# sea-sky-web/Vision-based-Spatio-Temporal-Analysis

Hardware: AMD Instinct MI355X
Metric: multi-cam frames/sec (7-cam→480×1440 BEV) (higher is better)
Workload: dtype f32; 1 GPU; 7-cam 1080x1920 -> resnet50(stride-8 features)+proj C=64 -> IPM warp -> mean -> 480x1440 BEV (BASELINE configs[1]); cameras=7, cameras_per_gpu=7, channels=64, bev_memory_format=NCHW, parallelism=frame-sharded x1 (no collective)

## Files before the change

include/bev_mi355x.h:

```cpp
#ifndef BEV_MI355X_H
#define BEV_MI355X_H

#include <stdint.h>

#ifdef __cplusplus
extern "C" {
#endif

#define BEV_ERR_ARGS (-1)

#define BEV_FUSE_SUM 0
#define BEV_FUSE_MEAN 1
#define BEV_FUSE_MAX 2

int bev_abi_version(void);

const char *bev_build_source_hash(void);

#define BEV_TUNE_CONV_TILE 1
#define BEV_TUNE_WARP_POOL_KB 2
#define BEV_TUNE_WARP_KERNEL 3
#define BEV_TUNE_WARP_BWD_POOL 5
#define BEV_TUNE_CONV_XCD 6
#define BEV_TUNE_CONV_NBUF 7
#define BEV_TUNE_WGRAD_MFMA 8
#define BEV_TUNE_CONV_DMA 9
#define BEV_TUNE_CONV_X6_TILE 10
#define BEV_TUNE_CONV_X6_KERNEL 11
#define BEV_TUNE_CONV_H16_KERNEL 12
#define BEV_TUNE_CONV_PW_SMALL 13
#define BEV_TUNE_DW_RUN 14
#define BEV_TUNE_CONV_X6_NT 16
#define BEV_TUNE_STEM3_STAGE 17
#define BEV_TUNE_WARP_SPAN 19
#define BEV_TUNE_WARP_TILE_BAND 20
#define BEV_TUNE_CONV_H16_BUF 21
int bev_tune(int knob, int value);


int bev_linspace_f32(double lo, double hi, int n, float *out_host);

int bev_homography_f32(const float *K, const float *G, int n, float *H, void *stream);


int bev_ipm_warp_f32(const float *feats, int64_t sN, int64_t sC, int64_t sH, int64_t sW, const float *Hmat,
                     const float *xs, const float *ys, int N, int C, int Hf, int Wf, float sx, float sy, int Hb,
                     int Wb, float *out, void *stream);

int bev_ipm_warp_fuse_f32(const float *feats, int64_t sN, int64_t sC, int64_t sH, int64_t sW, const float *Hmat,
                          const float *xs, const float *ys, int B, int V, int C, int Hf, int Wf, float sx, float sy,
                          int Hb, int Wb, int mode, float *out, void *stream);

int64_t bev_ipm_warp_fuse_workspace_bytes(int B, int V, int Hb, int Wb);
int bev_ipm_warp_fuse_ws_f32(const float *feats, int64_t sN, int64_t sC, int64_t sH, int64_t sW, const float *Hmat,
                             const float *xs, const float *ys, int B, int V, int C, int Hf, int Wf, float sx, float sy,
                             int Hb, int Wb, int mode, float *out, void *workspace, int64_t workspace_bytes,
                             void *stream);
int bev_ipm_warp_fuse_boxes_f32(const float *Hmat, const float *xs, const float *ys, int B, int V, int Hf, int Wf,
                                float sx, float sy, int Hb, int Wb, int mode, void *workspace, int64_t workspace_bytes,
                                void *stream);
int bev_ipm_warp_fuse_pre_f32(const float *feats, int64_t sN, int64_t sC, int64_t sH, int64_t sW, const float *Hmat,
                              const float *xs, const float *ys, int B, int V, int C, int Hf, int Wf, float sx, float sy,
                              int Hb, int Wb, int mode, float *out, void *workspace, int64_t workspace_bytes,
                              void *stream);
int bev_ipm_warp_fuse_nhwc_f32(const float *feats, int64_t sN, int64_t sC, int64_t sH, int64_t sW, const float *Hmat,
                               const float *xs, const float *ys, int B, int V, int C, int Hf, int Wf, float sx,
                               float sy, int Hb, int Wb, int mode, float *out, void *workspace,
                               int64_t workspace_bytes, int boxes_ready, void *stream);
int bev_ipm_warp_fuse_chunked_f32(const float *feats, int64_t sN, int64_t sC, int64_t sH, int64_t sW,
                                  const float *Hmat, const float *xs, const float *ys, int B, int V, int C, int Hf,
                                  int Wf, float sx, float sy, int Hb, int Wb, int mode, int rows_per_chunk, float *out,
                                  void *workspace, int64_t workspace_bytes, int boxes_ready, void *stream);

int bev_ipm_taps_f32(const float *Hmat, const float *xs, const float *ys, int N, int Hf, int Wf, float sx, float sy,
                     int Hb, int Wb, int32_t *x0y0, float *wts, uint8_t *valid, void *stream);

int bev_ipm_warp_bwd_f32(const float *gout, const float *Hmat, const float *xs, const float *ys, int N, int C, int Hf,
                         int Wf, float sx, float sy, int Hb, int Wb, float *gfeats, void *stream);

int bev_ipm_warp_bwd_ex_f32(const float *gout, const float *Hmat, const float *xs, const float *ys, int N, int C,
                            int Hf, int Wf, float sx, float sy, int Hb, int Wb, float *gfeats, int64_t sN, int64_t sC,
                            int64_t sH, int64_t sW, void *stream);

int bev_ipm_warp_fuse_bwd_f32(const float *gout, const float *Hmat, const float *xs, const float *ys, int B, int V,
                              int C, int Hf, int Wf, float sx, float sy, int Hb, int Wb, int mode, float *gfeats,
                              void *stream);

int bev_ipm_warp_fuse_bwd_ex_f32(const float *gout, const float *Hmat, const float *xs, const float *ys, int B,
                                 int V, int C, int Hf, int Wf, float sx, float sy, int Hb, int Wb, int mode,
                                 float *gfeats, int64_t sN, int64_t sC, int64_t sH, int64_t sW, void *stream);

int bev_view_fuse_f32(const float *x, int B, int V, int64_t M, int mode, float *out, void *stream);

int bev_view_max_bwd_f32(const float *x, const float *gout, int B, int V, int64_t M, float *gx, void *stream);


int64_t bev_conv_packed_size(int Co, int Ci, int KH, int KW);

int bev_conv_pack_weights_f32(const float *w, int Co, int Ci, int KH, int KW, float *packed, void *stream);

int bev_conv2d_f32(const float *x, int in_nchw, int N, int H, int W, int Ci, const float *packed, const float *bias,
                   const float *residual, int Co, int KH, int KW, int stride, int pad, int relu, float *y, int Ho,
                   int Wo, void *stream);

int bev_conv2d_chscale_f32(const float *x, int N, int H, int W, int Ci, const float *gate, const float *packed,
                           const float *bias, const float *residual, int Co, int KH, int KW, int stride, int pad,
                           int relu, float *y, int Ho, int Wo, void *stream);

int bev_conv2d_dual_f32(const float *x, int N, int Ho, int Wo, int Ci, const float *x2, int H2, int W2, int Ci2,
                        int stride2, const float *packed, const float *bias, int Co, int relu, float *y,
                        void *stream);

int bev_conv2d_chain_f32(const float *x, int N, int H, int W, int Ci, const float *packed, const float *bias, int Co,
                         int KH, int KW, int stride, int pad, int relu, const float *packed2, const float *bias2,
                         int Co2, const float *residual, int relu2, float *y, int Ho, int Wo, void *stream);

int bev_conv2d_chain_dual_f32(const float *x, int N, int H, int W, int Ci, const float *packed, const float *bias,
                              int Co, int KH, int KW, int stride, int pad, int relu, const float *x2, int H2, int W2,
                              int Ci2, int stride2, const float *packed2, const float *bias2, int Co2, int relu2,
// ... 297 lines not shown
```

vision-based-spatio-temporal-analysis_amd/bev_native.py:

```python
from __future__ import annotations

import collections.abc
import contextlib
import ctypes
import functools
import os
import subprocess
import threading

import torch

HERE = os.path.dirname(os.path.abspath(__file__))
LIB_PATH = os.path.join(HERE, "libbev_mi355x.so")
ABI_VERSION = 18
BEV_ERR_ARGS = -1

FUSE_MODES = {"sum": 0, "mean": 1, "max": 2}

_lib = None

_vp = ctypes.c_void_p
_i = ctypes.c_int
_i64 = ctypes.c_int64
_f = ctypes.c_float
# ... 164 lines not shown
    global _SPANS
    spans, _SPANS = _SPANS or {}, None
    torch.cuda.synchronize()
    return {k: [a.elapsed_time(b) for a, b in v] for k, v in spans.items()}


@contextlib.contextmanager
def _span(name: str, t: torch.Tensor):
    if _SPANS is None:
        yield
        return
    st = torch.cuda.current_stream(t.device)
    e0, e1 = torch.cuda.Event(enable_timing=True), torch.cuda.Event(enable_timing=True)
    e0.record(st)
    yield
    e1.record(st)
    _SPANS.setdefault(name, []).append((e0, e1))


def build(force: bool = False) -> str:
    cmd = ["make", "-s", "-C", HERE] + (["-B"] if force else [])
    subprocess.check_call(cmd)
    return LIB_PATH


def lib():
    global _lib
    if _lib is None:
        if not os.path.exists(LIB_PATH):
            raise ImportError(f"libbev_mi355x.so not built ({LIB_PATH}); run __graft_entry__.build()")
        L = ctypes.CDLL(LIB_PATH)
        for name, (res, args) in SIGNATURES.items():
            fn = getattr(L, name)
            fn.restype = res
            fn.argtypes = args
        v = L.bev_abi_version()
        if v != ABI_VERSION:
            raise ImportError(f"libbev_mi355x.so ABI {v} != expected {ABI_VERSION}; rebuild")
        _lib = L
    return _lib


def source_hash() -> str:
    import hashlib
    mk = open(os.path.join(HERE, "Makefile")).read()
    files = []
    for var in ("SRCS", "HDRS"):
        line = next(l for l in mk.splitlines() if l.startswith(var + " ="))
        files += line.split("=", 1)[1].split()
    h = hashlib.sha256()
    for f in files:
        with open(os.path.join(HERE, f), "rb") as fh:
            h.update(fh.read())
    return h.hexdigest()[:16]


def provenance() -> dict:
    built = lib().bev_build_source_hash().decode()
    try:
        tree = source_hash()
    except OSError:
        tree = None
    return {"lib": LIB_PATH, "lib_source_hash": built, "tree_source_hash": tree, "matches_tree": built == tree}


TUNE_CONV_TILE = 1
TUNE_WARP_POOL_KB = 2
TUNE_WARP_KERNEL = 3
TUNE_WARP_BWD_POOL = 5
TUNE_CONV_XCD = 6
TUNE_CONV_NBUF = 7
TUNE_WGRAD_MFMA = 8
TUNE_CONV_DMA = 9
TUNE_CONV_X6_TILE = 10
TUNE_CONV_X6_KERNEL = 11
TUNE_CONV_H16_KERNEL = 12
TUNE_CONV_PW_SMALL = 13
TUNE_DW_RUN = 14
TUNE_CONV_X6_NT = 16
TUNE_STEM3_STAGE = 17
TUNE_WARP_SPAN = 19
TUNE_WARP_TILE_BAND = 20
TUNE_CONV_H16_BUF = 21
WARP_KERNEL_DMA, WARP_KERNEL_REGISTER = 0, 1


def tune(knob: int, value: int) -> int:
    rc = lib().bev_tune(knob, value)
    if rc < 0:
        raise ValueError(f"bad tuning knob/value {knob}/{value}")
    return rc


@contextlib.contextmanager
def tuned(**knobs):
    old = []
    try:
        for name, value in knobs.items():
            k = globals()["TUNE_" + name]
            old.append((k, tune(k, value)))
        yield
    finally:
        for k, v in reversed(old):
            tune(k, v)


class HipError(RuntimeError):
    pass


AMP_HALF_CONVS = True
_AMP_LOCAL = threading.local()


CONV_ARITHS = ("f32", "bf16x6", "f16")
_ARITH = {"mode": "bf16x6"}


def conv_arith() -> str:
    return _ARITH["mode"]


def set_conv_arith(mode: str) -> str:
    if mode not in CONV_ARITHS:
        raise ValueError(f"conv arithmetic {mode!r} not in {CONV_ARITHS}")
    prev, _ARITH["mode"] = _ARITH["mode"], mode
    return prev


@contextlib.contextmanager
def conv_arith_mode(mode: str):
    prev = set_conv_arith(mode)
    try:
        yield
    finally:
        set_conv_arith(prev)


HEAD_ARITHS = ("f32", "f16")
_HEAD_ARITH = {"mode": "f32"}


def head_arith() -> str:
    return _HEAD_ARITH["mode"]


def set_head_arith(mode: str) -> str:
    if mode not in HEAD_ARITHS:
        raise ValueError(f"head arithmetic {mode!r} not in {HEAD_ARITHS}")
    prev, _HEAD_ARITH["mode"] = _HEAD_ARITH["mode"], mode
    return prev


@contextlib.contextmanager
def head_arith_mode(mode: str):
    prev = set_head_arith(mode)
    try:
        yield
    finally:
        set_head_arith(prev)


def half_convs() -> bool:
    return getattr(_AMP_LOCAL, "half", False)


# ... 1842 lines not shown
```

vision-based-spatio-temporal-analysis_amd/csrc/bev_conv.hip:

```cpp
#include <hip/hip_runtime.h>
#include <stdint.h>
#include <stdlib.h>

#include <type_traits>

#include "../../include/bev_mi355x.h"
#include "bev_act.h"
#include "bev_mfma.h"
#include "bev_tune.h"

namespace {

constexpr int BK = 32;
constexpr int LROW = BK + 4;

typedef float f32x16 __attribute__((ext_vector_type(16)));
typedef float f32x2 __attribute__((ext_vector_type(2)));
typedef float f32x4 __attribute__((ext_vector_type(4)));

__device__ __attribute__((aligned(16))) float g_zero4[4] = {0.f, 0.f, 0.f, 0.f};

__host__ __device__ inline int64_t kpad(int K) { return (K + BK - 1) / BK * BK; }
__host__ __device__ inline int64_t copad(int Co) { return (Co + 127) / 128 * 128; }

// ... 1189 lines not shown
        default: return false;
    }
    rc = last();
    return true;
}

int g_conv_tile = 0;

int g_conv_xcd = 1;
int g_conv_nbuf = 0;
inline int conv_xcd() { return g_conv_xcd; }

int launch_tiled(const ConvArgs &a, int loader, hipStream_t st) {
    int rc_pw = 0;
    if (g_conv_tile == 0 && try_pw_small(a, loader, st, rc_pw)) return rc_pw;
    if (g_conv_tile == 0 && try_pw_mfma(a, loader, st, rc_pw)) return rc_pw;
    const int64_t M = a.M;
    const int Co = a.Co;
    const int nbuf_env = g_conv_nbuf;
    auto nbuf1_for = [&](int tile) {
        if (nbuf_env == 1 || nbuf_env == 2) return nbuf_env == 1;
        return tile == 3 || M >= 400000;
    };
    int tile = g_conv_tile;
    if (tile == 0) {
        auto cost = [&](int bm, int bn, int resident) {
            const int64_t blocks = ((M + bm - 1) / bm) * ((Co + bn - 1) / bn);
            return (double)((blocks + resident - 1) / resident) * bm * bn;
        };
        const double c1 = cost(128, 128, 512), c3 = cost(64, 128, nbuf1_for(3) ? 768 : 512),
                     c2 = cost(128, 64, nbuf1_for(2) ? 768 : 512);
        tile = 1;
        double best = c1;
        if (c3 < 0.95 * best) { tile = 3; best = c3; }
        if (c2 < 0.95 * best) { tile = 2; best = c2; }
        if (a.KH == 1 && a.KW == 1 && (loader == 1 || loader == 6) && M >= 200000) tile = 4;
        if (a.KH == 1 && a.KW == 1 && loader == 4 && M >= 200000 && (Co <= 64 || a.Ci >= 48)) tile = 4;
    }
    if (tile == 2)
        return nbuf1_for(2) ? launch_conv<4, 1, 1, 2, 1>(a, loader, st) : launch_conv<4, 1, 1, 2>(a, loader, st);
    if (tile == 3)
        return nbuf1_for(3) ? launch_conv<2, 2, 1, 2, 1>(a, loader, st) : launch_conv<2, 2, 1, 2>(a, loader, st);
    if (tile == 4) return launch_conv<2, 2, 1, 1, 1>(a, loader, st);
    return launch_conv<2, 2, 2, 2>(a, loader, st);
}

int launch_chain(const ConvArgs &a, hipStream_t st) {
    const int bm = a.Co == 64 ? 128 : 64;
    const int64_t blocks = (a.M + bm - 1) / bm;
    if (blocks > 0x7fffffff) return BEV_ERR_ARGS;
    const dim3 g((unsigned)blocks), b(256);
    if (use_dma(a.Co)) {
        if (a.Co == 64) hipLaunchKernelGGL((k_conv_dma<4, 1, 1, 2, 1>), g, b, 0, st, a);
        else hipLaunchKernelGGL((k_conv_dma<2, 2, 1, 2, 1>), g, b, 0, st, a);
    } else if (a.Co == 64) hipLaunchKernelGGL((k_conv<4, 1, 1, 2, 1, 1, 1>), g, b, 0, st, a);
    else hipLaunchKernelGGL((k_conv<2, 2, 1, 2, 1, 1, 1>), g, b, 0, st, a);
    return last();
}

ConvArgs conv_args(const float *x, const float *packed, const float *bias, const float *res, float *y, int N, int H,
                   int W, int Ci, int Co, int KH, int KW, int stride, int pad, int dil, int Ho, int Wo, int relu,
                   int ldy) {
    ConvArgs a;
    a.x = x, a.wp = packed, a.bias = bias, a.res = res, a.y = y;
    a.N = N, a.H = H, a.W = W, a.Ci = Ci, a.Co = Co, a.KH = KH, a.KW = KW, a.stride = stride, a.pad = pad;
    a.dil = dil, a.Ho = Ho, a.Wo = Wo, a.relu = relu, a.ldy = ldy;
    a.M = (int64_t)N * Ho * Wo;
    a.K = Ci * KH * KW;
    a.Kp = (int)kpad(a.K);
    a.xcd = conv_xcd();
    return a;
}

}

extern "C" {

int bev_tune(int knob, int value) {
    if (knob == BEV_TUNE_CONV_TILE) return bev::swap_knob(g_conv_tile, value, 4);
    if (knob == BEV_TUNE_CONV_DMA) return bev::swap_knob(g_conv_dma, value, 2);
    if (knob == BEV_TUNE_CONV_XCD) return bev::swap_knob(g_conv_xcd, value, 1);
    if (knob == BEV_TUNE_CONV_NBUF) return bev::swap_knob(g_conv_nbuf, value, 2);
    if (knob == BEV_TUNE_WGRAD_MFMA) return bev::train_tune(knob, value);
    if (knob == BEV_TUNE_CONV_X6_TILE || knob == BEV_TUNE_CONV_X6_KERNEL || knob == BEV_TUNE_CONV_X6_NT)
        return bev::conv_x6_tune(knob, value);
    if (knob == BEV_TUNE_CONV_H16_KERNEL) return bev::conv_h16_tune(value);
    if (knob == BEV_TUNE_CONV_H16_BUF) return bev::conv_h16_buf_tune(value);
    if (knob == BEV_TUNE_DW_RUN) return bev::dw_tune(value);
    if (knob == BEV_TUNE_STEM3_STAGE) return bev::stem3_tune(value);
    if (knob == BEV_TUNE_CONV_PW_SMALL) return bev::swap_knob(g_conv_pw_small, value, 4);
    return bev::warp_tune(knob, value);
}

int64_t bev_conv_packed_size(int Co, int Ci, int KH, int KW) {
    if (Co <= 0 || Ci <= 0 || KH <= 0 || KW <= 0) return 0;
    return copad(Co) * kpad(Ci * KH * KW);
}

int bev_conv_pack_weights_f32(const float *w, int Co, int Ci, int KH, int KW, float *packed, void *stream) {
    if (!w || !packed || Co <= 0 || Ci <= 0 || KH <= 0 || KW <= 0) return BEV_ERR_ARGS;
    const int64_t Kp = kpad(Ci * KH * KW), Cop = copad(Co);
    const int64_t total = Kp * Cop;
    hipLaunchKernelGGL(k_pack, dim3((unsigned)((total + 255) / 256)), dim3(256), 0, (hipStream_t)stream, w, Co, Ci,
                       KH, KW, Kp, Cop, packed);
    return last();
}

static int conv2d_impl(const float *x, int in_nchw, int N, int H, int W, int Ci, const float *packed,
                       const float *bias, const float *residual, int Co, int KH, int KW, int stride, int pad, int relu,
                       float *y, int Ho, int Wo, const float *ascale, void *stream, int dil, int ldy,
                       const float *ashift, int arelu);

int bev_conv2d_f32(const float *x, int in_nchw, int N, int H, int W, int Ci, const float *packed, const float *bias,
                   const float *residual, int Co, int KH, int KW, int stride, int pad, int relu, float *y, int Ho,
                   int Wo, void *stream) {
    return conv2d_impl(x, in_nchw, N, H, W, Ci, packed, bias, residual, Co, KH, KW, stride, pad, relu, y, Ho, Wo,
                       nullptr, stream, 1, Co, nullptr, 0);
}

int bev_conv2d_nhwc_ex_f32(const float *x, int N, int H, int W, int Ci, const float *in_scale, const float *in_shift,
                           int in_relu, const float *packed, const float *bias, int Co, int KH, int KW, int stride,
                           int pad, int dilation, int relu, float *y, int ldy, int Ho, int Wo, void *stream) {
    if ((in_shift || in_relu) && !in_scale) return BEV_ERR_ARGS;
    if (in_scale && (Ci % BK != 0 || ((((uintptr_t)in_scale) | ((uintptr_t)in_shift) | ((uintptr_t)x)) & 15) != 0))
        return BEV_ERR_ARGS;
    return conv2d_impl(x, 0, N, H, W, Ci, packed, bias, nullptr, Co, KH, KW, stride, pad, relu, y, Ho, Wo, in_scale,
                       stream, dilation, ldy, in_shift, in_relu != 0);
}

int bev_conv2d_chscale_f32(const float *x, int N, int H, int W, int Ci, const float *gate, const float *packed,
                           const float *bias, const float *residual, int Co, int KH, int KW, int stride, int pad,
                           int relu, float *y, int Ho, int Wo, void *stream) {
    if (!gate || ((((uintptr_t)gate) | ((uintptr_t)x)) & 15) != 0 || Ci % 4 != 0) return BEV_ERR_ARGS;
    const bool fast = Ci % BK == 0;
    const bool contig = KH == 1 && KW == 1 && stride == 1 && pad == 0;
    if (!fast && !contig) return BEV_ERR_ARGS;
    return conv2d_impl(x, 0, N, H, W, Ci, packed, bias, residual, Co, KH, KW, stride, pad, relu, y, Ho, Wo, gate,
                       stream, 1, Co, nullptr, 0);
}

static int conv2d_impl(const float *x, int in_nchw, int N, int H, int W, int Ci, const float *packed,
                       const float *bias, const float *residual, int Co, int KH, int KW, int stride, int pad, int relu,
                       float *y, int Ho, int Wo, const float *ascale, void *stream, int dil, int ldy,
                       const float *ashift, int arelu) {
    if (!x || !packed || !y || N < 0 || H <= 0 || W <= 0 || Ci <= 0 || Co <= 0 || KH <= 0 || KW <= 0 ||
        stride <= 0 || pad < 0 || relu < 0 || relu > 2 || dil <= 0 || ldy < Co || (residual && ldy != Co))
        return BEV_ERR_ARGS;
    if (Ho != conv_out(H, pad, dil, KH, stride) || Wo != conv_out(W, pad, dil, KW, stride) ||
        Ho <= 0 || Wo <= 0)
        return BEV_ERR_ARGS;
    if (N == 0) return 0;
    ConvArgs a = conv_args(x, packed, bias, residual, y, N, H, W, Ci, Co, KH, KW, stride, pad, dil, Ho, Wo, relu, ldy);
    a.in_nchw = in_nchw;
    const bool pw = !in_nchw && KH == 1 && KW == 1 && stride == 1 && pad == 0 && Ci % 4 == 0 &&
                    ((uintptr_t)x & 15) == 0;
    int loader = (!in_nchw && Ci % BK == 0) ? 1 : (in_nchw && Ci == 3 && KH == 7 && KW == 7) ? 2 : pw ? 4 : 0;
    if (loader == 1 && (ashift || arelu || dil != 1)) loader = 5;
    else if (loader == 1 && ascale) loader = 6;
    if ((ashift || arelu) && loader != 5) return BEV_ERR_ARGS;
    a.ascale = ascale;
    a.ashift = ashift;
    a.arelu = arelu;
    if (in_nchw && Ci == 3 && KH == 7 && KW == 7 && stride == 2 && pad == 3 && Co <= 64 && !residual && bias &&
        g_conv_tile == 0 && relu <= 1 && !ascale && dil == 1 && ldy == Co)
        return launch_stem(x, N, H, W, packed, a.Kp, bias, Co, y, Ho, Wo, relu, (hipStream_t)stream);
    return launch_tiled(a, loader, (hipStream_t)stream);
}
// ... 169 lines not shown
```

vision-based-spatio-temporal-analysis_amd/csrc/bev_conv_x6.hip:

```cpp
#include <hip/hip_runtime.h>
#include <stdint.h>

#include <type_traits>

#include "../../include/bev_mi355x.h"
#include "bev_act.h"
#include "bev_mfma.h"
#include "bev_tune.h"

namespace {

typedef __bf16 bf16x8 __attribute__((ext_vector_type(8)));
typedef __bf16 bf16x4 __attribute__((ext_vector_type(4)));
typedef float f32x16 __attribute__((ext_vector_type(16)));
typedef float f32x4 __attribute__((ext_vector_type(4)));
typedef unsigned u32x4 __attribute__((ext_vector_type(4)));
typedef unsigned u32x2 __attribute__((ext_vector_type(2)));

constexpr int XBK = 16;
constexpr int XROW = 24;

__device__ __attribute__((aligned(16))) float g_xzero4[4] = {0.f, 0.f, 0.f, 0.f};

__host__ __device__ inline int64_t kpad_x(int K) { return (K + XBK - 1) / XBK * XBK; }
// ... 611 lines not shown
            *(bf16x4 *)(d + 2 * APL) = lv;                                                                 \
        }                                                                                                  \
    } while (0)
#define X6B_BLOAD(BS, G)                                                                                   \
    do {                                                                                                   \
        const int g_ = (G) < nslice ? (G) : nslice - 1;              \
        _Pragma("unroll") for (int j = 0; j < TN; ++j)                                                     \
            _Pragma("unroll") for (int p = 0; p < 3; ++p)                                                  \
                BS[j][p] = *(const bf16x8 *)(wb + ((int64_t)j * S + g_) * 1536 + p * 512);                \
    } while (0)
    const int r32 = lane & 31, h = lane >> 5;
#define X6B_SLICE(AS, KK, BC)                                                                              \
    do {                                                                                                   \
        bf16x8 fa[TM][3];                                                                                  \
        _Pragma("unroll") for (int i = 0; i < TM; ++i)                                                     \
            _Pragma("unroll") for (int p = 0; p < 3; ++p)                                                  \
                fa[i][p] = *(const bf16x8 *)(AS + p * APL + (wm * TM * 32 + i * 32 + r32) * YROW + 16 * (KK) + 8 * h); \
        _Pragma("unroll") for (int i = 0; i < TM; ++i)                                                     \
            _Pragma("unroll") for (int j = 0; j < TN; ++j)                                                 \
                x6_dot(acc[i][j], fa[i], BC[j]);                                                           \
    } while (0)
#define X6B_MFMA(BUF, KS)                                                                                  \
    do {                                                                                                   \
        const __bf16 *As = lds + (BUF) * STAGE;                                                            \
        X6B_SLICE(As, 0, bs0);                                                                             \
        X6B_BLOAD(bs0, 2 * (KS) + 2);                                                                      \
        X6B_SLICE(As, 1, bs1);                                                                             \
    } while (0)

    const int nk = a.Kp / YBK;
    X6B_BLOAD(bs0, 0);
    X6B_GLOAD(va0);
    if (nk > 1) X6B_GLOAD(va1);
    X6B_SWRITE(0, va0);
    __syncthreads();
    int ks = 0;
    for (; ks + 3 < nk; ks += 2) {
        X6B_BLOAD(bs1, 2 * ks + 1);
        X6B_GLOAD(va0);
        X6B_MFMA(0, ks);
        X6B_SWRITE(1, va1);
        __syncthreads();
        X6B_BLOAD(bs1, 2 * ks + 3);
        X6B_GLOAD(va1);
        X6B_MFMA(1, ks + 1);
        X6B_SWRITE(0, va0);
        __syncthreads();
    }
    if (ks + 2 < nk) {
        X6B_BLOAD(bs1, 2 * ks + 1);
        X6B_GLOAD(va0);
        X6B_MFMA(0, ks);
        X6B_SWRITE(1, va1);
        __syncthreads();
        X6B_BLOAD(bs1, 2 * ks + 3);
        X6B_MFMA(1, ks + 1);
        X6B_SWRITE(0, va0);
        __syncthreads();
        X6B_BLOAD(bs1, 2 * ks + 5);
        X6B_MFMA(0, ks + 2);
    } else if (ks + 1 < nk) {
        X6B_BLOAD(bs1, 2 * ks + 1);
        X6B_MFMA(0, ks);
        X6B_SWRITE(1, va1);
        __syncthreads();
        X6B_BLOAD(bs1, 2 * ks + 3);
        X6B_MFMA(1, ks + 1);
    } else {
        X6B_BLOAD(bs1, 2 * ks + 1);
        X6B_MFMA(0, ks);
    }
#undef X6B_MFMA
#undef X6B_SLICE
#undef X6B_BLOAD
#undef X6B_SWRITE
#undef X6B_GLOAD
    if constexpr (CHAIN > 0) {
        x6_chain_epilogue<WM, WN, TM, TN, CHAIN == 2 ? 4 : 0>(a, lds_raw, acc, wave, lane, wm, wn, m0);
        return;
    }
    x6_epilogue<TM, TN>(a, (float *)lds_raw, acc, wave, lane, wn, wm, m0, n0);
}

template <int WM, int WN, int TM, int TN, int CHAIN = 0>
__global__ __launch_bounds__(256, CHAIN ? 2 : 3) void k_conv_x6s(ConvX a) {
    constexpr bool BLDS = CHAIN > 0;
    constexpr int BM = WM * TM * 32, BN = WN * TN * 32;
    constexpr int APL = BM * 32;
    constexpr int BST = BLDS ? BN / 32 * 6 * 512 : 0;
    constexpr int STAGE = 3 * APL + BST;
    constexpr int RW = BM / 4;
    constexpr int RG = RW / 16;
    constexpr int BPW = BLDS ? BN / 32 * 6 / 4 : 0;
    constexpr int EPIB = CHAIN ? x6_chain_lds_bytes<BM, BN>() : x6_epi_bytes<TN>();
    constexpr int LDSB = (2 * STAGE * 2 > EPIB) ? 2 * STAGE * 2 : EPIB;
    static_assert(RW % 16 == 0, "whole DMA groups per wave");
    static_assert(!BLDS || (BN / 32 * 6) % 4 == 0, "whole B pieces per wave");
    __shared__ __attribute__((aligned(16))) unsigned char lds_raw[LDSB];
    const __bf16 *lds = (const __bf16 *)lds_raw;

    const int tid = threadIdx.x;
    const int lane = tid & 63, wave = __builtin_amdgcn_readfirstlane(tid >> 6);
    const int wm = wave / WN, wn = wave % WN;
    const int n_tiles = (a.Co + BN - 1) / BN;
    const unsigned bid = xcd_block(blockIdx.x, gridDim.x);
    const int64_t m0 = (int64_t)(bid / n_tiles) * BM;
    const int n0 = (bid % n_tiles) * BN;

    int64_t abase[RG];
    int aiy[RG], aix[RG];
    bool aok[RG];
#pragma unroll
    for (int g = 0; g < RG; ++g) {
        const int row = wave * RW + 16 * g + (lane >> 2);
        const int lc = (lane & 3) ^ ((row >> 2) & 3);
        const int64_t m = m0 + row;
        aok[g] = m < a.M;
        const int64_t mm = aok[g] ? m : 0;
        const int ox = (int)(mm % a.Wo);
        const int64_t t = mm / a.Wo;
        const int oy = (int)(t % a.Ho);
        const int64_t n = t / a.Ho;
        aiy[g] = oy * a.stride - a.pad;
        aix[g] = ox * a.stride - a.pad;
        abase[g] = ((n * a.H + aiy[g]) * a.W + aix[g]) * a.Ci + 8 * lc;
    }
    const unsigned lbase = (unsigned)__builtin_amdgcn_readfirstlane((int)lds_addr(lds_raw));
    const int S = a.Kp / XBK;
    int ky = 0, kx = 0, ci0 = 0, kstep = 0;
    const __bf16 *bsrc = a.wp + (int64_t)(n0 >> 5) * S * 1536 + lane * 8;
    auto issue = [&](int buf) {
        if constexpr (BLDS) {
            const unsigned db = lbase + (unsigned)(buf * STAGE * 2 + 3 * APL * 2);
#pragma unroll
            for (int i = 0; i < BPW; ++i) {
                const int q = wave + 4 * i, cbl = q / 6, r = q % 6;
                lds_dma16(bsrc + ((int64_t)cbl * S + 2 * kstep + r / 3) * 1536 + (r % 3) * 512,
                      db + (unsigned)(q * 1024));
            }
            ++kstep;
        }
        const int64_t toff = ((int64_t)ky * a.dil * a.W + kx * a.dil) * a.Ci + ci0;
        const unsigned d0 = lbase + (unsigned)(buf * STAGE * 2) + (unsigned)(wave * RW * 64);
#pragma unroll
        for (int g = 0; g < RG; ++g) {
            const int iy = aiy[g] + ky * a.dil, ix = aix[g] + kx * a.dil;
            const bool in = aok[g] && (unsigned)iy < (unsigned)a.H && (unsigned)ix < (unsigned)a.W;
            const __bf16 *src = a.xs + abase[g] + toff;
#pragma unroll
            for (int p = 0; p < 3; ++p)
                lds_dma16(in ? (const void *)(src + p * a.xps) : (const void *)g_xzero4,
                      d0 + (unsigned)(p * APL * 2 + g * 1024));
        }
        ci0 += YBK;
        if (ci0 == a.Ci) {
            ci0 = 0;
            if (++kx == a.KW) {
                kx = 0;
                ++ky;
            }
        }
    };

    const __amdgpu_buffer_rsrc_t rw = buffer_rsrc(a.wp, copad_x(a.Co) / 32 * (int64_t)S * 3072);
    const int cb0 = (n0 + wn * TN * 32) >> 5;
    const int vl = lane * 16;
    bf16x8 bs0[TN][3], bs1[TN][3];
#define X6S_BLOAD(BS, G)                                                                                   \
    do {                                                                                                   \
        const int g_ = (G) < S ? (G) : S - 1;                                                              \
        _Pragma("unroll") for (int j = 0; j < TN; ++j)                                                     \
            _Pragma("unroll") for (int p = 0; p < 3; ++p)                                                  \
                BS[j][p] = __builtin_bit_cast(                                                             \
                    bf16x8, __builtin_amdgcn_raw_buffer_load_b128(rw, vl, (((cb0 + j) * S + g_) * 3 + p) * 1024, 0)); \
    } while (0)
    const int r32 = lane & 31, h = lane >> 5;
#define X6S_SLICE(AS, KK, BC)                                                                              \
    do {                                                                                                   \
        bf16x8 fa[TM][3];                                                                                  \
        _Pragma("unroll") for (int i = 0; i < TM; ++i) {                                                   \
            const int R = wm * TM * 32 + i * 32 + r32;                                                     \
            const int ph = (2 * (KK) + h) ^ ((R >> 2) & 3);                                                \
            _Pragma("unroll") for (int p = 0; p < 3; ++p)                                                  \
                fa[i][p] = *(const bf16x8 *)(AS + p * APL + R * 32 + ph * 8);                              \
        }                                                                                                  \
        _Pragma("unroll") for (int i = 0; i < TM; ++i)                                                     \
            _Pragma("unroll") for (int j = 0; j < TN; ++j)                                                 \
                x6_dot(acc[i][j], fa[i], BC[j]);                                                           \
    } while (0)

    f32x16 acc[TM][TN];
#pragma unroll
    for (int i = 0; i < TM; ++i)
#pragma unroll
        for (int j = 0; j < TN; ++j) acc[i][j] = (f32x16){0};
    const int nk = a.Kp / YBK;
    if constexpr (BLDS) {
        issue(0);
        asm volatile("s_waitcnt vmcnt(0)" ::: "memory");
        __syncthreads();
        for (int ks = 0; ks < nk; ++ks) {
            const int cur = ks & 1;
            if (ks + 1 < nk) issue(cur ^ 1);
            const __bf16 *As = lds + cur * STAGE;
            const __bf16 *Bs = As + 3 * APL + lane * 8;
#pragma unroll
            for (int kk = 0; kk < 2; ++kk) {
                bf16x8 fb[TN][3];
#pragma unroll
                for (int j = 0; j < TN; ++j)
#pragma unroll
                    for (int p = 0; p < 3; ++p) fb[j][p] = *(const bf16x8 *)(Bs + (((wn * TN + j) * 2 + kk) * 3 + p) * 512);
                X6S_SLICE(As, kk, fb);
            }
            asm volatile("s_waitcnt vmcnt(0)" ::: "memory");
            __syncthreads();
        }
    } else {
        X6S_BLOAD(bs0, 0);
        issue(0);
        asm volatile("s_waitcnt vmcnt(0)" ::: "memory");
        __syncthreads();
        for (int ks = 0; ks < nk; ++ks) {
            const int cur = ks & 1;
            if (ks + 1 < nk) issue(cur ^ 1);
            const __bf16 *As = lds + cur * STAGE;
            X6S_BLOAD(bs1, 2 * ks + 1);
            X6S_SLICE(As, 0, bs0);
            X6S_BLOAD(bs0, 2 * ks + 2);
            X6S_SLICE(As, 1, bs1);
            asm volatile("s_waitcnt vmcnt(0)" ::: "memory");
            __syncthreads();
        }
    }
#undef X6S_SLICE
#undef X6S_BLOAD
    if constexpr (CHAIN > 0) {
        x6_chain_epilogue<WM, WN, TM, TN, CHAIN == 2 ? 4 : 0>(a, lds_raw, acc, wave, lane, wm, wn, m0);
        return;
    }
    x6_epilogue<TM, TN>(a, (float *)lds_raw, acc, wave, lane, wn, wm, m0, n0);
}

__global__ void k_split3(const float *__restrict__ x, int64_t n, __bf16 *__restrict__ out) {
    const int64_t t = (int64_t)blockIdx.x * blockDim.x + threadIdx.x;
    if (t >= n) return;
    __bf16 h, m, l;
    split3(x[t], h, m, l);
    out[t] = h;
    out[t + n] = m;
    out[t + 2 * n] = l;
}

int g_x6_tile = 0;
int g_x6_nt = 0;
int g_x6_kernel = 0;

int launch_x6(void (*kernel)(ConvX), int BM, int BN, const ConvX &a, hipStream_t st) {
    const int64_t blocks = ((a.M + BM - 1) / BM) * ((a.Co + BN - 1) / BN);
    if (blocks >= ((int64_t)1 << 31)) return BEV_ERR_ARGS;
    hipLaunchKernelGGL(kernel, dim3((unsigned)blocks), dim3(256), 0, st, a);
    return last();
}

enum X6Form { X6_PLAIN, X6_DUAL, X6_CHAIN, X6_CHAIN_DUAL };
struct X6Call {
    X6Form form;
    const float *x = nullptr;
    const uint16_t *xs = nullptr, *packed = nullptr;
    const float *bias = nullptr, *res = nullptr;
    float *y = nullptr;
    uint16_t *ys = nullptr;
    int N = 0, H = 0, W = 0, Ci = 0, Co = 0, KH = 1, KW = 1, stride = 1, pad = 0, dil = 1, act = 0, ldy = 0, Ho = 0,
        Wo = 0;
    const float *x2 = nullptr;
    int H2 = 0, W2 = 0, Ci2 = 0, stride2 = 0;
    const uint16_t *packed2 = nullptr;
    const float *bias2 = nullptr;
    int Co2 = 0, act2 = 0;
};

int conv_x6(const X6Call &c, hipStream_t st) {
    const bool chain = c.form == X6_CHAIN || c.form == X6_CHAIN_DUAL;
    const bool second = c.form == X6_DUAL || c.form == X6_CHAIN_DUAL;
    if ((!c.x == !c.xs) || !c.packed || (!c.y == !c.ys) || c.N < 0 || c.H <= 0 || c.W <= 0 || c.Co <= 0 || c.KH <= 0 ||
        c.KW <= 0 || c.stride <= 0 || c.pad < 0 || c.dil <= 0 || c.act < 0 || c.act > 2)
        return BEV_ERR_ARGS;
    if ((!chain && c.Ci <= 0) || c.Ci % (chain || c.xs ? YBK : XBK) != 0) return BEV_ERR_ARGS;
    if (second && (!c.x2 || c.H2 <= 0 || c.W2 <= 0 || c.Ci2 <= 0 || c.stride2 <= 0)) return BEV_ERR_ARGS;
    if (c.form == X6_DUAL && c.Ci2 % XBK != 0) return BEV_ERR_ARGS;
    if (chain && (!c.packed2 || c.act2 < 0 || c.act2 > 2 || c.Co2 <= 0 || c.Co2 % 64 != 0)) return BEV_ERR_ARGS;
    if (c.form == X6_CHAIN && c.Co != 64 && c.Co != 128) return BEV_ERR_ARGS;
    if (c.form == X6_CHAIN_DUAL && (c.Co != 64 || c.Ci2 != 64)) return BEV_ERR_ARGS;
    if (c.Ho != conv_out(c.H, c.pad, c.dil, c.KH, c.stride) || c.Wo != conv_out(c.W, c.pad, c.dil, c.KW, c.stride) ||
        c.Ho <= 0 || c.Wo <= 0)
        return BEV_ERR_ARGS;
    if (second && (c.Ho != conv_out(c.H2, 0, 1, 1, c.stride2) || c.Wo != conv_out(c.W2, 0, 1, 1, c.stride2)))
        return BEV_ERR_ARGS;
    if ((((uintptr_t)c.x | (uintptr_t)c.xs | (uintptr_t)c.x2 | (uintptr_t)c.packed | (uintptr_t)c.packed2) & 15) != 0)
        return BEV_ERR_ARGS;
    if (!chain && (c.ldy < c.Co || (c.res && c.ldy != c.Co))) return BEV_ERR_ARGS;
    if (c.ys && (c.ldy != c.Co || c.Co % 4 != 0 || ((uintptr_t)c.ys & 7) != 0)) return BEV_ERR_ARGS;
    if (c.N == 0) return 0;
    if (c.form == X6_CHAIN && c.Co != 64 && c.Co2 % 128 != 0) return BEV_ERR_ARGS;

    ConvX a;
    a.x = c.x, a.wp = (const __bf16 *)c.packed, a.bias = c.bias, a.res = c.res, a.y = c.y;
    a.N = c.N, a.H = c.H, a.W = c.W, a.Ci = c.Ci, a.Co = c.Co, a.KH = c.KH, a.KW = c.KW, a.stride = c.stride;
    a.pad = c.pad, a.dil = c.dil, a.Ho = c.Ho, a.Wo = c.Wo, a.act = c.act, a.ldy = chain ? c.Co2 : c.ldy;
    a.Kp = (int)kpad_x(c.form == X6_DUAL ? c.Ci + c.Ci2 : c.Ci * c.KH * c.KW);
    a.M = (int64_t)c.N * c.Ho * c.Wo;
    a.x2 = c.x2, a.Ci2 = c.Ci2, a.H2 = c.H2, a.W2 = c.W2, a.stride2 = c.stride2;
    a.xs = (const __bf16 *)c.xs, a.ys = (__bf16 *)c.ys;
    a.xps = (int64_t)c.N * c.H * c.W * c.Ci, a.yps = a.M * c.Co;
    a.wp2 = (const __bf16 *)c.packed2, a.bias2 = c.bias2, a.Co2 = c.Co2, a.act2 = c.act2;

    if (c.form == X6_CHAIN_DUAL)
        return launch_x6(c.xs ? k_conv_x6s<4, 1, 1, 2, 2> : k_conv_x6b<4, 1, 1, 2, false, 2>, 128, 64, a, st);
    if (c.form == X6_CHAIN && c.Co == 64)
        return launch_x6(c.xs ? k_conv_x6s<4, 1, 1, 2, 1> : k_conv_x6b<4, 1, 1, 2, false, 1>, 128, 64, a, st);
    if (c.form == X6_CHAIN)
        return launch_x6(c.xs ? k_conv_x6s<2, 2, 1, 2, 1> : k_conv_x6b<2, 2, 1, 2, false, 1>, 64, 128, a, st);
    const bool dual = c.form == X6_DUAL;
    a.nta = g_x6_nt;
    const int t = g_x6_tile ? g_x6_tile : (a.Co <= 64 ? 2 : 1);
    if (a.xs) return t == 2 ? launch_x6(k_conv_x6s<4, 1, 1, 2>, 128, 64, a, st)
                            : launch_x6(k_conv_x6s<2, 2, 2, 2>, 128, 128, a, st);
    const bool wide = a.Ci % YBK == 0 && (!dual || a.Ci2 % YBK == 0) && g_x6_kernel != 1;
    if (wide && t == 2 && !dual && a.nta) return launch_x6(k_conv_x6b<4, 1, 1, 2, false, 0, true>, 128, 64, a, st);
    if (wide && t == 2)
        return launch_x6(dual ? k_conv_x6b<4, 1, 1, 2, true> : k_conv_x6b<4, 1, 1, 2, false>, 128, 64, a, st);
    if (wide) return launch_x6(dual ? k_conv_x6b<2, 2, 2, 2, true> : k_conv_x6b<2, 2, 2, 2, false>, 128, 128, a, st);
    if (t == 2) return launch_x6(dual ? k_conv_x6<4, 1, 1, 2, true> : k_conv_x6<4, 1, 1, 2, false>, 128, 64, a, st);
    return launch_x6(dual ? k_conv_x6<2, 2, 2, 2, true> : k_conv_x6<2, 2, 2, 2, false>, 128, 128, a, st);
}

namespace stem6 {
constexpr int TW = 64, TH = 8, NTHR = 512;
constexpr int PR = 2 * TH + 5;
constexpr int PC = 2 * TW + 5;
constexpr int PITCH = 136;
constexpr int PLANE = 3 * PR * PITCH;
constexpr int PER_T = 17;
constexpr int NRUN = 3 * 7;
constexpr int NS = (NRUN + 2) / 2;
constexpr int WB = 2 * NS * 3 * 512;
constexpr int S_PANEL = 10;
__host__ __device__ constexpr int roff(int run) { return run >= NRUN ? 0 : ((run % 3) * PR + run / 3) * PITCH; }
static_assert(PITCH >= 2 * TW + 6 && PITCH % 2 == 0, "slot 7 of the last output column inside the row");
static_assert(4 * 34 * 64 * 4 <= 3 * PLANE * 2, "the pool epilogue's row exchange fits in the patch");
}

struct StemX6Args {
    const float *__restrict__ x;
    const __bf16 *__restrict__ wp;
    const float *__restrict__ bias;
    float *__restrict__ y;
    int H, W, Co, Ho, Wo, relu, nTx, nTy;
    int64_t ntiles;
    float *__restrict__ edge_b, *__restrict__ edge_r;
    int Hp, Wp;
};

__device__ __forceinline__ unsigned stem6_fetch(const StemX6Args &a, int64_t t, int tid, float (&pv)[stem6::PER_T]) {
    using namespace stem6;
    const int tx = (int)(t % a.nTx);
    const int64_t r_ = t / a.nTx;
    const int ty = (int)(r_ % a.nTy);
    const int64_t img = r_ / a.nTy;
    const int row0 = 2 * ty * TH - 3, col0 = 2 * tx * TW - 3;
    const float *xi = a.x + img * 3 * (int64_t)a.H * a.W;
    unsigned in = 0;
#pragma unroll
    for (int i = 0; i < PER_T; ++i) {
        const int cr = i < PER_T - 1 ? (tid >> 7) + 4 * i : tid >> 3;
        const int c = i < PER_T - 1 ? (tid & 127) : 2 * TW + (tid & 7);
        const int ci = (cr >= PR) + (cr >= 2 * PR), r = cr - ci * PR;
        const int gy = row0 + r, gx = col0 + c;
        const bool ok = cr < 3 * PR && c < PC && (unsigned)gy < (unsigned)a.H && (unsigned)gx < (unsigned)a.W;
        pv[i] = xi[ok ? ((int64_t)ci * a.H + gy) * a.W + gx : 0];
        in |= (unsigned)ok << i;
    }
    return in;
}

__device__ __forceinline__ void stem6_put(__bf16 *pl, int tid, const float (&pv)[stem6::PER_T], unsigned in) {
    using namespace stem6;
    __bf16 *q = pl + (tid >> 7) * PITCH + (tid & 127);
#pragma unroll
    for (int i = 0; i < PER_T; ++i) {
        const bool last = i == PER_T - 1;
        if (last ? (tid >> 3) < 3 * PR && (tid & 7) < PC - 2 * TW : i < PER_T - 2 || (tid >> 7) < 3 * PR - 4 * i) {
            __bf16 *o = last ? pl + (tid >> 3) * PITCH + 2 * TW + (tid & 7) : q + 4 * i * PITCH;
            __bf16 hh, mm, ll;
            split3((in >> i) & 1u ? pv[i] : 0.0f, hh, mm, ll);
            o[0] = hh;
            o[PLANE] = mm;
            o[2 * PLANE] = ll;
        }
    }
}
// ... 181 lines not shown
                            }
                }
            }
        } else {
            const int tx = (int)(t % a.nTx);
            const int64_t r_ = t / a.nTx;
            const int ty = (int)(r_ % a.nTy);
            const int64_t img = r_ / a.nTy;
            const int oy = ty * TH + wave;
            const int oxb = tx * TW;
            __syncthreads();
            stem6_put(pl, tid, pv, pin);
            if (oy < a.Ho) {
                float *yr = a.y + ((img * a.Ho + oy) * (int64_t)a.Wo) * a.Co;
#pragma unroll
                for (int mt = 0; mt < 2; ++mt)
#pragma unroll
                    for (int r = 0; r < 16; ++r) {
                        const int ox = oxb + 32 * mt + (r & 3) + 8 * (r >> 2) + 4 * h;
                        if (ox < a.Wo) {
                            float v0 = acc[mt][0][r] + b0, v1 = acc[mt][1][r] + b1;
                            if (a.relu) {
                                v0 = relu_f(v0);
                                v1 = relu_f(v1);
                            }
                            float *yp = yr + (int64_t)ox * a.Co;
                            if (r32 < a.Co) yp[r32] = v0;
                            if (32 + r32 < a.Co) yp[32 + r32] = v1;
                        }
                    }
            }
        }
        __syncthreads();
    }
}

__global__ __launch_bounds__(256) void k_stem_pool_seams(float *__restrict__ y, const float *__restrict__ edge_b,
                                                         const float *__restrict__ edge_r, int nTx, int nTy,
                                                         int64_t ntiles, int Hp, int Wp) {
    const int64_t g = (int64_t)blockIdx.x * 256 + threadIdx.x;
    const int64_t tile = g / (35 * 16);
    if (tile >= ntiles) return;
    const int k = (int)(g - tile * (35 * 16)), s = k >> 4, c4 = k & 15;
    const int tx = (int)(tile % nTx);
    const int64_t r_ = tile / nTx;
    const int ty = (int)(r_ % nTy);
    const int64_t img = r_ / nTy;
    const int p = s < 32 ? 0 : s - 31, q = s < 32 ? s : 0;
    const int P = ty * (stem6::TH / 2) + p, Q = tx * (stem6::TW / 2) + q;
    if (P >= Hp || Q >= Wp || (p == 0 && ty == 0 && (q > 0 || tx == 0))) return;
    float4 *yp = reinterpret_cast<float4 *>(y + (((img * Hp + P) * (int64_t)Wp + Q) * 64)) + c4;
    float4 m = *yp;
    auto mx = [](float4 a, float4 b) {
        return make_float4(pool_mx(a.x, b.x), pool_mx(a.y, b.y), pool_mx(a.z, b.z), pool_mx(a.w, b.w));
    };
    if (p == 0 && ty > 0) m = mx(m, reinterpret_cast<const float4 *>(edge_b + ((tile - nTx) * 32 + q) * 64)[c4]);
    if (q == 0 && tx > 0) {
        m = mx(m, reinterpret_cast<const float4 *>(edge_r + ((tile - 1) * 5 + p) * 64)[c4]);
        if (p == 0 && ty > 0)
            m = mx(m, reinterpret_cast<const float4 *>(edge_r + ((tile - nTx - 1) * 5 + 4) * 64)[c4]);
    }
    *yp = m;
}

StemX6Args stem_x6_args(const float *x, int N, int H, int W, const uint16_t *packed, const float *bias, int Co,
                        int relu, float *y, int Ho, int Wo) {
    StemX6Args a;
    a.x = x, a.wp = (const __bf16 *)packed, a.bias = bias, a.y = y;
    a.H = H, a.W = W, a.Co = Co, a.Ho = Ho, a.Wo = Wo, a.relu = relu;
    a.nTx = (Wo + stem6::TW - 1) / stem6::TW;
    a.nTy = (Ho + stem6::TH - 1) / stem6::TH;
    a.ntiles = (int64_t)N * a.nTx * a.nTy;
    a.edge_b = a.edge_r = nullptr;
    a.Hp = a.Wp = 0;
    return a;
}
unsigned stem_x6_grid(const StemX6Args &a) { return (unsigned)(a.ntiles < cu_count() ? a.ntiles : cu_count()); }

}

namespace bev {
int conv_x6_tune(int knob, int value) {
    if (knob == BEV_TUNE_CONV_X6_TILE) return swap_knob(g_x6_tile, value, 2);
    return swap_knob(knob == BEV_TUNE_CONV_X6_NT ? g_x6_nt : g_x6_kernel, value, 1);
}
}

extern "C" {

int64_t bev_conv_packed_size_x6(int Co, int Ci, int KH, int KW) {
    if (Co <= 0 || Ci <= 0 || KH <= 0 || KW <= 0) return BEV_ERR_ARGS;
    return copad_x(Co) * kpad_x(Ci * KH * KW) * 3;
}

int bev_conv_pack_weights_x6(const float *w, int Co, int Ci, int KH, int KW, uint16_t *packed, void *stream) {
    if (!w || !packed || Co <= 0 || Ci <= 0 || KH <= 0 || KW <= 0) return BEV_ERR_ARGS;
    const int64_t Kp = kpad_x(Ci * KH * KW), Cop = copad_x(Co), n = Kp * Cop;
    hipLaunchKernelGGL(k_pack_x6, dim3((unsigned)((n + 255) / 256)), dim3(256), 0, (hipStream_t)stream, w, Co, Ci, KH,
                       KW, Kp, Cop, (__bf16 *)packed);
    return last();
}

int bev_conv2d_x6_f32(const float *x, const uint16_t *xs, int N, int H, int W, int Ci, const uint16_t *packed,
                      const float *bias, const float *residual, int Co, int KH, int KW, int stride, int pad,
                      int dilation, int act, float *y, uint16_t *ys, int ldy, int Ho, int Wo, void *stream) {
    X6Call c{X6_PLAIN};
    c.x = x, c.xs = xs, c.packed = packed, c.bias = bias, c.res = residual, c.y = y, c.ys = ys;
    c.N = N, c.H = H, c.W = W, c.Ci = Ci, c.Co = Co, c.KH = KH, c.KW = KW, c.stride = stride, c.pad = pad;
    c.dil = dilation, c.act = act, c.ldy = ldy, c.Ho = Ho, c.Wo = Wo;
    return conv_x6(c, (hipStream_t)stream);
}

int bev_split3_f32(const float *x, int64_t n, uint16_t *planes, void *stream) {
    if (!x || !planes || n < 0) return BEV_ERR_ARGS;
    if (n == 0) return 0;
    hipLaunchKernelGGL(k_split3, dim3((unsigned)((n + 255) / 256)), dim3(256), 0, (hipStream_t)stream, x, n,
                       (__bf16 *)planes);
    return last();
}

int bev_conv2d_dual_x6_f32(const float *x, int N, int Ho, int Wo, int Ci, const float *x2, int H2, int W2, int Ci2,
                           int stride2, const uint16_t *packed, const float *bias, int Co, int act, float *y,
                           void *stream) {
    X6Call c{X6_DUAL};
    c.x = x, c.packed = packed, c.bias = bias, c.y = y;
    c.N = N, c.H = c.Ho = Ho, c.W = c.Wo = Wo, c.Ci = Ci, c.Co = c.ldy = Co, c.act = act;
    c.x2 = x2, c.H2 = H2, c.W2 = W2, c.Ci2 = Ci2, c.stride2 = stride2;
    return conv_x6(c, (hipStream_t)stream);
}

int bev_conv2d_chain_x6_f32(const float *x, const uint16_t *xs, int N, int H, int W, int Ci,
                            const uint16_t *packed, const float *bias, int Co, int KH, int KW, int stride, int pad,
                            int act, const uint16_t *packed2, const float *bias2, int Co2, const float *residual,
                            int act2, float *y, int Ho, int Wo, void *stream) {
    X6Call c{X6_CHAIN};
    c.x = x, c.xs = xs, c.packed = packed, c.bias = bias, c.res = residual, c.y = y;
    c.N = N, c.H = H, c.W = W, c.Ci = Ci, c.Co = Co, c.KH = KH, c.KW = KW, c.stride = stride, c.pad = pad;
    c.act = act, c.Ho = Ho, c.Wo = Wo;
    c.packed2 = packed2, c.bias2 = bias2, c.Co2 = Co2, c.act2 = act2;
    return conv_x6(c, (hipStream_t)stream);
}

int bev_conv2d_chain_dual_x6_f32(const float *x, const uint16_t *xs, int N, int H, int W, int Ci,
                                 const uint16_t *packed, const float *bias, int Co, int KH, int KW, int stride,
                                 int pad, int act, const float *x2, int H2, int W2, int Ci2, int stride2,
                                 const uint16_t *packed2, const float *bias2, int Co2, int act2, float *y, int Ho,
                                 int Wo, void *stream) {
    X6Call c{X6_CHAIN_DUAL};
    c.x = x, c.xs = xs, c.packed = packed, c.bias = bias, c.y = y;
    c.N = N, c.H = H, c.W = W, c.Ci = Ci, c.Co = Co, c.KH = KH, c.KW = KW, c.stride = stride, c.pad = pad;
    c.act = act, c.Ho = Ho, c.Wo = Wo;
    c.x2 = x2, c.H2 = H2, c.W2 = W2, c.Ci2 = Ci2, c.stride2 = stride2;
    c.packed2 = packed2, c.bias2 = bias2, c.Co2 = Co2, c.act2 = act2;
    return conv_x6(c, (hipStream_t)stream);
}

int bev_conv2d_stem_x6_f32(const float *x, int N, int H, int W, const uint16_t *packed, const float *bias, int Co,
                           int relu, float *y, int Ho, int Wo, void *stream) {
    if (!x || !packed || !bias || !y || N <= 0 || H <= 0 || W <= 0 || Co <= 0 || Co > 64 ||
        Ho != conv_out(H, 3, 1, 7, 2) || Wo != conv_out(W, 3, 1, 7, 2) || (((uintptr_t)packed) & 15) != 0)
        return BEV_ERR_ARGS;
    const StemX6Args a = stem_x6_args(x, N, H, W, packed, bias, Co, relu, y, Ho, Wo);
    hipLaunchKernelGGL(k_stem_x6<false>, dim3(stem_x6_grid(a)), dim3(stem6::NTHR), 0, (hipStream_t)stream, a);
    return last();
}

// ... 29 lines not shown
```

Before: 141.4 frames/s.

## Add strip-reuse mainloop for 3x3 stride-1 chained x6 split-precision convs

Adds a specialized mainloop for 3x3/stride1/pad1 convs with 64 input channels in the 128x64 chained x6s kernels. It loads one contiguous row strip per ky into LDS, covering the 128-pixel tile plus halo, and reuses it across the three kx taps by shifting the row index. Image-edge columns are zeroed in registers instead of gathering each im2col row separately. This cuts redundant global/DMA loads of the activation but uses more LDS, which may lower occupancy. It is enabled by default and can be turned off with a new tune knob.

```diff
diff --git a/include/bev_mi355x.h b/include/bev_mi355x.h
--- a/include/bev_mi355x.h
+++ b/include/bev_mi355x.h
@@ -35,6 +35,7 @@
 #define BEV_TUNE_WARP_SPAN 19
 #define BEV_TUNE_WARP_TILE_BAND 20
 #define BEV_TUNE_CONV_H16_BUF 21
+#define BEV_TUNE_CONV_X6_STRIP 22
 int bev_tune(int knob, int value);
 
 
diff --git a/vision-based-spatio-temporal-analysis_amd/bev_native.py b/vision-based-spatio-temporal-analysis_amd/bev_native.py
--- a/vision-based-spatio-temporal-analysis_amd/bev_native.py
+++ b/vision-based-spatio-temporal-analysis_amd/bev_native.py
@@ -270,6 +270,7 @@
 TUNE_WARP_SPAN = 19
 TUNE_WARP_TILE_BAND = 20
 TUNE_CONV_H16_BUF = 21
+TUNE_CONV_X6_STRIP = 22
 WARP_KERNEL_DMA, WARP_KERNEL_REGISTER = 0, 1
 
 
diff --git a/vision-based-spatio-temporal-analysis_amd/csrc/bev_conv.hip b/vision-based-spatio-temporal-analysis_amd/csrc/bev_conv.hip
--- a/vision-based-spatio-temporal-analysis_amd/csrc/bev_conv.hip
+++ b/vision-based-spatio-temporal-analysis_amd/csrc/bev_conv.hip
@@ -1295,7 +1295,8 @@
     if (knob == BEV_TUNE_CONV_XCD) return bev::swap_knob(g_conv_xcd, value, 1);
     if (knob == BEV_TUNE_CONV_NBUF) return bev::swap_knob(g_conv_nbuf, value, 2);
     if (knob == BEV_TUNE_WGRAD_MFMA) return bev::train_tune(knob, value);
-    if (knob == BEV_TUNE_CONV_X6_TILE || knob == BEV_TUNE_CONV_X6_KERNEL || knob == BEV_TUNE_CONV_X6_NT)
+    if (knob == BEV_TUNE_CONV_X6_TILE || knob == BEV_TUNE_CONV_X6_KERNEL || knob == BEV_TUNE_CONV_X6_NT ||
+        knob == BEV_TUNE_CONV_X6_STRIP)
         return bev::conv_x6_tune(knob, value);
     if (knob == BEV_TUNE_CONV_H16_KERNEL) return bev::conv_h16_tune(value);
     if (knob == BEV_TUNE_CONV_H16_BUF) return bev::conv_h16_buf_tune(value);
diff --git a/vision-based-spatio-temporal-analysis_amd/csrc/bev_conv_x6.hip b/vision-based-spatio-temporal-analysis_amd/csrc/bev_conv_x6.hip
--- a/vision-based-spatio-temporal-analysis_amd/csrc/bev_conv_x6.hip
+++ b/vision-based-spatio-temporal-analysis_amd/csrc/bev_conv_x6.hip
@@ -717,7 +717,106 @@
     x6_epilogue<TM, TN>(a, (float *)lds_raw, acc, wave, lane, wn, wm, m0, n0);
 }
 
-template <int WM, int WN, int TM, int TN, int CHAIN = 0>
+__device__ __forceinline__ void x6s_strip_mainloop(const ConvX &a, unsigned char *lds_raw, f32x16 (&acc)[1][2],
+                                                   int wave, int lane, int64_t m0) {
+    constexpr int SROWS = 144, SUSED = 130;
+    constexpr int SPL = SROWS * 32;
+    constexpr int HSB = 3 * SPL * 2;
+    constexpr int BSTB = 2 * 6 * 1024;
+    constexpr int NPC = 27;
+    constexpr int NP = (NPC + 3) / 4;
+    constexpr int YOUT = -(1 << 30);
+    const __bf16 *lds = (const __bf16 *)lds_raw;
+    const unsigned lbase = (unsigned)__builtin_amdgcn_readfirstlane((int)lds_addr(lds_raw));
+    const int r32 = lane & 31, h = lane >> 5;
+
+    const int lc = (lane & 3) ^ ((lane >> 4) & 3);
+    const int64_t loff = (m0 - 1 + (lane >> 2)) * 64 + 8 * lc;
+    int yv[NP];
+#pragma unroll
+    for (int i = 0; i < NP; ++i) {
+        const int g = (wave + 4 * i) % 9;
+        const int sr = 16 * g + (lane >> 2);
+        const int64_t p = m0 - 1 + sr;
+        const bool ok = sr < SUSED && p >= 0 && p < a.M;
+        yv[i] = ok ? (int)((p / a.W) % a.H) : YOUT;
+    }
+    auto issue_strip = [&](int half, int ky) {
+        const int64_t so = (int64_t)(ky - 1) * a.W * 64 + half * 32;
+        const unsigned d0 = lbase + (unsigned)(half * HSB);
+#pragma unroll
+        for (int i = 0; i < NP; ++i) {
+            const int q = wave + 4 * i;
+            if (q < NPC) {
+                const int pl = q / 9, g = q % 9;
+                const bool in = (unsigned)(yv[i] + ky - 1) < (unsigned)a.H;
+                const __bf16 *src = a.xs + (loff + so + (int64_t)g * (16 * 64) + pl * a.xps);
+                lds_dma16(in ? (const void *)src : (const void *)g_xzero4, d0 + (unsigned)(pl * SPL * 2 + g * 1024));
+            }
+        }
+    };
+    const int S = a.Kp / XBK;
+    const __bf16 *bsrc = a.wp + lane * 8;
+    int kstep = 0;
+    auto issue_b = [&](int buf) {
+        const unsigned db = lbase + (unsigned)(2 * HSB + buf * BSTB);
+#pragma unroll
+        for (int i = 0; i < 3; ++i) {
+            const int q = wave + 4 * i, cbl = q / 6, r = q % 6;
+            lds_dma16(bsrc + ((int64_t)cbl * S + 2 * kstep + r / 3) * 1536 + (r % 3) * 512, db + (unsigned)(q * 1024));
+        }
+        ++kstep;
+    };
+
+    const int R = wave * 32 + r32;
+    const int ox = (int)((m0 + R) % a.W);
+    const bool e0 = ox == 0, e2 = ox == a.W - 1;
+    const bool any0 = __builtin_amdgcn_ballot_w64(e0) != 0, any2 = __builtin_amdgcn_ballot_w64(e2) != 0;
+
+    issue_b(0);
+    issue_strip(0, 0);
+    asm volatile("s_waitcnt vmcnt(0)" ::: "memory");
+    __syncthreads();
+    for (int ky = 0; ky < 3; ++ky) {
+#pragma unroll
+        for (int t = 0; t < 6; ++t) {
+            const int kx = t >> 1, half = t & 1;
+            if (t < 5 || ky < 2) issue_b((t + 1) & 1);
+            if (t == 0) issue_strip(1, ky);
+            if (t == 5 && ky < 2) issue_strip(0, ky + 1);
+            const __bf16 *As = lds + half * (3 * SPL);
+            const __bf16 *Bs = (const __bf16 *)(lds_raw + 2 * HSB + (t & 1) * BSTB) + lane * 8;
+            const int r = R + kx;
+#pragma unroll
+            for (int kk = 0; kk < 2; ++kk) {
+                bf16x8 fb[2][3], fa[3];
+#pragma unroll
+                for (int j = 0; j < 2; ++j)
+#pragma unroll
+                    for (int p = 0; p < 3; ++p) fb[j][p] = *(const bf16x8 *)(Bs + ((j * 2 + kk) * 3 + p) * 512);
+                const int ph = (2 * kk + h) ^ ((r >> 2) & 3);
+#pragma unroll
+                for (int p = 0; p < 3; ++p) fa[p] = *(const bf16x8 *)(As + p * SPL + r * 32 + ph * 8);
+                if ((kx == 0 && any0) || (kx == 2 && any2)) {
+                    const bool z = kx == 0 ? e0 : e2;
+#pragma unroll
+                    for (int p = 0; p < 3; ++p) {
+                        u32x4 v = __builtin_bit_cast(u32x4, fa[p]);
+#pragma unroll
+                        for (int e = 0; e < 4; ++e) v[e] = z ? 0u : v[e];
+                        fa[p] = __builtin_bit_cast(bf16x8, v);
+                    }
+                }
+#pragma unroll
+                for (int j = 0; j < 2; ++j) x6_dot(acc[0][j], fa, fb[j]);
+            }
+            asm volatile("s_waitcnt vmcnt(0)" ::: "memory");
+            __syncthreads();
+        }
+    }
+}
+
+template <int WM, int WN, int TM, int TN, int CHAIN = 0, bool STRIP = false>
 __global__ __launch_bounds__(256, CHAIN ? 2 : 3) void k_conv_x6s(ConvX a) {
     constexpr bool BLDS = CHAIN > 0;
     constexpr int BM = WM * TM * 32, BN = WN * TN * 32;
@@ -728,9 +827,11 @@
     constexpr int RG = RW / 16;
     constexpr int BPW = BLDS ? BN / 32 * 6 / 4 : 0;
     constexpr int EPIB = CHAIN ? x6_chain_lds_bytes<BM, BN>() : x6_epi_bytes<TN>();
-    constexpr int LDSB = (2 * STAGE * 2 > EPIB) ? 2 * STAGE * 2 : EPIB;
+    constexpr int MAINB = STRIP ? 2 * (3 * 144 * 64) + 2 * BST * 2 : 2 * STAGE * 2;
+    constexpr int LDSB = (MAINB > EPIB) ? MAINB : EPIB;
     static_assert(RW % 16 == 0, "whole DMA groups per wave");
     static_assert(!BLDS || (BN / 32 * 6) % 4 == 0, "whole B pieces per wave");
+    static_assert(!STRIP || (CHAIN > 0 && WM == 4 && WN == 1 && TM == 1 && TN == 2), "strip: the 128 x 64 chains");
     __shared__ __attribute__((aligned(16))) unsigned char lds_raw[LDSB];
     const __bf16 *lds = (const __bf16 *)lds_raw;
 
@@ -741,6 +842,13 @@
     const unsigned bid = xcd_block(blockIdx.x, gridDim.x);
     const int64_t m0 = (int64_t)(bid / n_tiles) * BM;
     const int n0 = (bid % n_tiles) * BN;
+
+    if constexpr (STRIP) {
+        f32x16 sacc[1][2] = {{(f32x16){0}, (f32x16){0}}};
+        x6s_strip_mainloop(a, lds_raw, sacc, wave, lane, m0);
+        x6_chain_epilogue<WM, WN, TM, TN, CHAIN == 2 ? 4 : 0>(a, lds_raw, sacc, wave, lane, wm, wn, m0);
+        return;
+    }
 
     int64_t abase[RG];
     int aiy[RG], aix[RG];
@@ -890,6 +998,7 @@
 int g_x6_tile = 0;
 int g_x6_nt = 0;
 int g_x6_kernel = 0;
+int g_x6_strip = 1;
 
 int launch_x6(void (*kernel)(ConvX), int BM, int BN, const ConvX &a, hipStream_t st) {
     const int64_t blocks = ((a.M + BM - 1) / BM) * ((a.Co + BN - 1) / BN);
@@ -950,8 +1059,12 @@
     a.xps = (int64_t)c.N * c.H * c.W * c.Ci, a.yps = a.M * c.Co;
     a.wp2 = (const __bf16 *)c.packed2, a.bias2 = c.bias2, a.Co2 = c.Co2, a.act2 = c.act2;
 
+    const bool strip = g_x6_strip && c.xs && c.KH == 3 && c.KW == 3 && c.stride == 1 && c.pad == 1 && c.dil == 1 &&
+                       c.Ci == 64;
+    if (c.form == X6_CHAIN_DUAL && strip) return launch_x6(k_conv_x6s<4, 1, 1, 2, 2, true>, 128, 64, a, st);
     if (c.form == X6_CHAIN_DUAL)
         return launch_x6(c.xs ? k_conv_x6s<4, 1, 1, 2, 2> : k_conv_x6b<4, 1, 1, 2, false, 2>, 128, 64, a, st);
+    if (c.form == X6_CHAIN && c.Co == 64 && strip) return launch_x6(k_conv_x6s<4, 1, 1, 2, 1, true>, 128, 64, a, st);
     if (c.form == X6_CHAIN && c.Co == 64)
         return launch_x6(c.xs ? k_conv_x6s<4, 1, 1, 2, 1> : k_conv_x6b<4, 1, 1, 2, false, 1>, 128, 64, a, st);
     if (c.form == X6_CHAIN)
@@ -1299,6 +1412,7 @@
 namespace bev {
 int conv_x6_tune(int knob, int value) {
     if (knob == BEV_TUNE_CONV_X6_TILE) return swap_knob(g_x6_tile, value, 2);
+    if (knob == BEV_TUNE_CONV_X6_STRIP) return swap_knob(g_x6_strip, value, 1);
     return swap_knob(knob == BEV_TUNE_CONV_X6_NT ? g_x6_nt : g_x6_kernel, value, 1);
 }
 }
```

Result: faster. 144.5 frames/s, median of 6 (+2.2%).
